# Gadersd/whisper-burn

Hardware: AMD Instinct MI355X
Metric: real-time factor (audio-sec/wall-sec) (higher is better)
Workload: dtype f32; 1 GPU; tiny.en, 30 s of 16 kHz audio per GPU per step, reference windowing (3 windows <= 14.9 s, 3 s overlap), HIP mel + encoder + KV-cached decode, greedy (beam_size 1), max_depth 100; windows=3, beam_size=1, max_depth=100, encoder_gemm_after_the_run=f16x3, parallelism=windows sharded over 1 GPU(s), 1 token all-gather

## Files before the change

### profiles/ps_timeline.py

```python
#!/usr/bin/env python3
import sys

import numpy as np

raw = np.fromfile(sys.argv[1], dtype=np.uint8)
n_steps, n_roles, grid, ns = [int(x) for x in raw[:16].view(np.int32)]
kinds = raw[16:16 + 4 * n_roles].view(np.int32)
n_st = 8 * n_steps * n_roles * ns
st = raw[16 + 4 * n_roles:16 + 4 * n_roles + n_st].view(np.uint64).reshape(n_steps, n_roles, ns).astype(np.float64)
tail = raw[16 + 4 * n_roles + n_st:]
block = None
if len(tail) >= 4 * (grid + 2) and int(tail[:4].view(np.int32)[0]) == 0x66664f52:
    role_off = tail[4:4 * (grid + 2)].view(np.int32)
    block = np.searchsorted(role_off, np.arange(n_roles), side="right") - 1
st[st == 0] = np.nan
names = {0: "attn", 1: "cross", 2: "mlp", 3: "logits", 4: "merge", 5: "finln"}
kind, layer, row = kinds & 0xff, (kinds >> 8) & 0xff, kinds >> 16
ran = ~np.isnan(st[:, :, 6])
last = int(np.nonzero(ran.any(1))[0].max()) + 1 if ran.any() else 0
lo = int(sys.argv[2]) if len(sys.argv) > 2 else min(8, max(last - 1, 0))
hi = int(sys.argv[3]) if len(sys.argv) > 3 else last
live_row = int(sys.argv[4]) if len(sys.argv) > 4 else 0
tick = 0.01
print(f"steps stamped {last} of {n_steps}, roles/step {n_roles}, grid {grid}; statistics over steps [{lo}, {hi}), attention roles of row {live_row}")
# ... 13 lines not shown
            continue
        s = sel[:, cols, :]
        def d(a, b):
            x = (s[:, :, b] - s[:, :, a]) * tick
            return np.nanmean(x) if np.isfinite(x).any() else float("nan")
        rel_done = np.nanmean((np.nanmax(s[:, :, 6], axis=1) - step_start) * tick)
        rel_arr = np.nanmean((np.nanmax(s[:, :, 7], axis=1) - step_start) * tick)
        nm = names[k] + (f" L{l}" if k < 3 else "")
        if k in (0, 1, 3, 4, 5):
            wp = np.nanmean((s[:, :, 1] - step_start[:, None]) * tick, axis=0)
            dn = np.nanmean((s[:, :, 6] - step_start[:, None]) * tick, axis=0)
            spread.append((nm, wp, dn, block[cols] if block is not None else None))
        print(f"{nm:<10}{int(cols.sum()):>4}{d(0,1):>8.2f}{d(1,2):>8.2f}{d(2,3):>8.2f}{d(3,4):>8.2f}{d(4,5):>8.2f}{d(5,6):>9.2f}{d(6,7):>8.2f}{d(1,6):>8.2f}{rel_done:>9.2f}{rel_arr:>9.2f}")
dd = np.diff(step_end) * tick
print(f"step time (merge arrived -> next merge arrived): mean {np.nanmean(dd):.2f} us, median {np.nanmedian(dd):.2f}, min {np.nanmin(dd):.2f}, max {np.nanmax(dd):.2f}")
print("over the roles of a kind (each role: mean over the steps), us after the step start (merge: of its own step's start):")
print(f"{'role':<10}{'n':>4}  {'wait passed @  min / median / max':<36}{'done @  min / median / max':<34}")
for nm, wp, dn, blk in spread:
    f3 = lambda v: f"{np.nanmin(v):8.2f} /{np.nanmedian(v):8.2f} /{np.nanmax(v):8.2f}"
    print(f"{nm:<10}{len(wp):>4}  {f3(wp):<36}{f3(dn):<34}")
    if nm == "logits" and blk is not None:
        late = np.argsort(-np.nan_to_num(dn))[:12]
        def held(b):
            o = [names[kind[i]] + f" L{layer[i]}" for i in np.nonzero(block == b)[0] if kind[i] < 3]
            return "+".join(o) if o else "-"
        print(f"{'':<10}last to finish (block [its layer roles]: wait passed @ / done @)  " +
              "  ".join(f"b{blk[i]}[{held(blk[i])}]:{wp[i]:.2f}/{dn[i]:.2f}" for i in late))
        behind = np.array([held(b) != "-" for b in blk])
        for lab, m in (("behind a layer role", behind), ("on blocks without one", ~behind)):
            if m.any():
# ... 5 lines not shown
```

### whisper-burn_amd/csrc/decode.h

```cpp
#pragma once
#include <hip/hip_runtime.h>
#include <hip/hip_ext.h>
#include <stdint.h>

#include <algorithm>
#include <vector>

#include "kernels.h"
#include "wb_internal.h"

namespace wb {

constexpr int MAX_BEAMS = 8;
constexpr int TOPK_MAX = 8;
constexpr int CA_STRIDE = 66;
constexpr int CA_NCH_MAX = 12;
constexpr int TS_STRIDE = 2 + 2 * TOPK_MAX;
constexpr int GV_CT = 128;
constexpr int GV_CT_LOGITS = 128;
constexpr int KS_MAX = 16;

enum { ST_N = 0, ST_STEP = 1, ST_HDR = 4 };
enum { GC_STEP = 0, GC_NDONE = 1, GC_ALLDONE = 2, GC_BAD = 3, GC_HDR = 4 };
struct StepLayout {
// ... 308 lines not shown
  const PsRole* roles = nullptr; int n_roles = 0;
  const int* role_off = nullptr;
  const int* res_role = nullptr;
  int n_logits_roles = 0;
  int n_layer = 0, n_rows = 0, S = 0, d = 0, n_head = 0, nb_mlp = 0;
  int n_pass = 1;
  int* ctl = nullptr;
  int step0 = 0, n_steps = 0;
  int n_forced = 0; int forced[PS_MAX_FORCED] = {0, 0, 0, 0, 0, 0, 0, 0};
  int mask_until_len = 0;
  const void* x_fin = nullptr; const void* P2 = nullptr; const float* b2_last = nullptr;
  void* g_xn = nullptr;
  unsigned tag_base = 0;
  const float* ln_g = nullptr; const float* ln_b = nullptr; float ln_eps = 0.f; int ln_inside = 0;
  const float* Et = nullptr; int vocab_ld = 0, V = 0; const float* mask = nullptr;
  float* tstats = nullptr; int n_tiles = 0;
  int* gctl = nullptr; int* gtok = nullptr; int Lmax = 0, eot = 0;
  const float* E = nullptr; const float* pos = nullptr; void* x0 = nullptr; int* tabs = nullptr;
  int* dead = nullptr;
  unsigned long long* stamps = nullptr;
};
enum { PS_DEAL_SLACK = 0, PS_DEAL_LEGACY = 1 };
struct PsDeal {
  std::vector<PsRole> roles;
  std::vector<int> role_off;
  std::vector<int> res_role;
  int n_lg = 0, n_res = 0;
};
PsDeal ps_deal_roles(int n_layer, int n_head, int n_rows, int nb_mlp, int n_tiles, int grid, int policy, bool res_on);
int ps_ctl_ints(int S, int n_layer);
bool dec_persist_supported(int d, int n_rows, int max_keys);
int dec_persist_resident_slots(int d, int n_rows, int max_keys);
bool dec_persist_resident_geometry(int d, int n_rows, int max_keys, int out[5]);
int dec_persist_max_grid(int device, int d, int n_rows, int max_keys);
int launch_dec_persist(hipStream_t st, const PersistArgs& a, int grid);
void launch_ps_seed(hipStream_t st, const float* x, int n, void* gx, unsigned tag, int* ctl);

#if defined(HIPEMU) && !defined(HIPEMU_PROD_GEOMETRY)
constexpr int CROSS_FUSED_MAX_C = 384;
#else
constexpr int CROSS_FUSED_MAX_C = 768;
#endif
constexpr int CROSS_FUSED_MAX_PASSES = 2;
void launch_dec_cross_fused(hipStream_t st, const CrossFusedArgs& a, int n_rows_hint);
bool dec_fused_supported(int d);
int dec_mlp_fused_planes(int d);
void launch_dec_mlp_fused(hipStream_t st, const MlpFusedArgs& a, int n_rows_hint);
void launch_dec_attn_fused(hipStream_t st, const AttnFusedArgs& a, int n_rows_hint);
int launch_dec_attn_fused_rounds(hipStream_t st, const AttnFusedArgs& a, int n_rows_hint, int n_reg);

}
// ... 1 lines not shown
```

### whisper-burn_amd/csrc/decode_chain.cpp

```cpp
#include <climits>
#include <cstring>
#include <string>

#include "decode_step.h"
#include "handoff.h"
#include "switches.h"

using namespace wb;

namespace wb {

struct PsPin { size_t seed, err, gctl, tok, total, ctl_ints; };
static PsPin ps_pin_layout(size_t ctl_ints, size_t tok_ints) {
  PsPin p;
  p.seed = 0; p.err = (ctl_ints + 3) & ~(size_t)3; p.gctl = p.err + 4; p.tok = p.gctl + ((ctl_ints + 3) & ~(size_t)3);
  p.total = p.tok + tok_ints; p.ctl_ints = ctl_ints;
  return p;
}
static int ps_pin_ensure(wb_session* s, size_t ints) {
  if (s->ps_pin_ints >= ints) return WB_OK;
  if (s->ps_pin_busy) { WB_HIP(hipStreamSynchronize(s->st)); s->ps_pin_busy = false; }
  if (s->ps_pin) { (void)hipHostFree(s->ps_pin); s->ps_pin = nullptr; s->ps_pin_ints = 0; }
  WB_HIP(hipHostMalloc((void**)&s->ps_pin, ints * 4, hipHostMallocDefault));
  s->ps_pin_ints = ints;
// ... 180 lines not shown
  WB_REQUIRE(n_forced >= 0 && n_forced <= PS_MAX_FORCED, WB_ERR_ARG, "persistent decode: %d prompt steps", n_forced);
  const char* inject = sw::persist_inject_fail();
  wb_model* m = s->m;
  const wb_dims& D = m->dims;
  const int d = D.n_text_state, H = D.n_text_head, NL = D.n_text_layer, V = D.n_vocab, S = s->S, W = s->W;
  const StepLayout& L = s->lay;
  hipStream_t st = s->st;
  const int NB = dec_mlp_fused_planes(d);
  const int n_tiles = (V + 127) / 128;
  WB_REQUIRE(NB <= 32 && H <= 8, WB_ERR_SHAPE, "persistent decode: more planes than its folds hold");
  WB_TRY(s->ps_gx.ensure_zeroed(((size_t)2 * S + 8) * d * 8, st));
  WB_TRY(s->ps_gpa.ensure_zeroed(((size_t)H * S + 8) * d * 8, st));
  WB_TRY(s->ps_gpc.ensure_zeroed(((size_t)H * S + 8) * d * 8, st));
  WB_TRY(s->ps_gp2.ensure_zeroed(((size_t)NB * S + 8) * d * 8, st));
  WB_TRY(s->ps_gxn.ensure_zeroed(((size_t)S + 8) * d * 8, st));
  if (((s->ps_launches + 1) & 0xffffu) == 0) {
    for (DevMem* b : {&s->ps_gx, &s->ps_gpa, &s->ps_gpc, &s->ps_gp2, &s->ps_gxn}) WB_HIP(hipMemsetAsync(b->p, 0, b->bytes, st));
    s->ps_launches++;
  }
  const unsigned tag_base = ((++s->ps_launches) & 0xffffu) << 16;
  char* gxb[2] = {static_cast<char*>(s->ps_gx.p), static_cast<char*>(s->ps_gx.p) + (size_t)S * d * 8};
  const char* res_sw = sw::persist_resident();
  const bool res_on = !(res_sw && res_sw[0] == '0') && dec_persist_resident_slots(d, W, s->maxC) > 0;
  bool built = false;
  WB_TRY(ps_setup_ensure(s, res_on, &built));
  const std::vector<PsRole>& roles = s->ps_roles_host;
  const int grid = s->ps_setup_grid, n_res = s->ps_setup_n_res;
  if (res_sw && !strcmp(res_sw, "log")) fprintf(stderr, "persist resident blocks: %d of %d\n", n_res, grid);
  const int n_ctl = ps_ctl_ints(S, NL);
  WB_TRY(s->ps_ctl.ensure((size_t)n_ctl * 4));
  WB_TRY(s->ps_dead.ensure((size_t)S * 4));
  WB_TRY(s->ps_tstats.ensure((size_t)S * n_tiles * 2 * 4));
  WB_HIP(hipMemsetAsync(s->ps_ctl.p, 0, (size_t)n_ctl * 4, st));
  WB_HIP(hipMemsetAsync(s->ps_dead.p, 0, (size_t)S * 4, st));
  PersistArgs a;
  a.layers = s->ps_layers.as<PsLayerArgs>(); a.roles = s->ps_roles.as<PsRole>(); a.n_roles = (int)roles.size();
  a.role_off = reinterpret_cast<const int*>(static_cast<char*>(s->ps_roles.p) + roles.size() * sizeof(PsRole));
  if (n_res > 0) a.res_role = a.role_off + (grid + 1);
  a.n_logits_roles = s->ps_setup_n_lg;
  a.n_layer = NL; a.n_rows = W; a.S = S; a.d = d; a.n_head = H; a.nb_mlp = NB;
  a.n_pass = s->maxC > CROSS_FUSED_MAX_C ? 2 : 1;
  a.ctl = s->ps_ctl.as<int>(); a.step0 = s->step; a.n_steps = n_forced + max_depth; a.mask_until_len = mask_until_len;
  a.n_forced = n_forced;
  for (int i = 0; i < n_forced; i++) a.forced[i] = forced[i];
  a.g_xn = s->ps_gxn.p;
  a.x_fin = gxb[(3 * NL) & 1]; a.P2 = s->ps_gp2.p; a.b2_last = m->dec[NL - 1].mlp2.b; a.tag_base = tag_base;
  a.ln_g = m->ln_dec.g; a.ln_b = m->ln_dec.b; a.ln_eps = m->ln_dec.eps; a.ln_inside = m->ln_eps_inside_sqrt;
  a.Et = m->tok_emb_t; a.vocab_ld = m->vocab_ld; a.V = V; a.mask = s->mask.as<float>();
  a.tstats = s->ps_tstats.as<float>(); a.n_tiles = n_tiles;
  a.gctl = s->gctl.as<int>(); a.gtok = s->gtok.as<int>(); a.Lmax = s->Lmax; a.eot = eot;
  a.E = m->tok_emb; a.pos = m->dec_pos; a.x0 = gxb[0]; a.tabs = s->tabs.as<int>(); a.dead = s->ps_dead.as<int>();
  const char* stamps_path = sw::ps_stamps();
  const size_t n_stamps = stamps_path ? (size_t)(n_forced + max_depth) * roles.size() * 8 : 0;
  if (n_stamps) {
    WB_TRY(s->ps_stamps.ensure(n_stamps * 8));
    WB_HIP(hipMemsetAsync(s->ps_stamps.p, 0, n_stamps * 8, st));
    a.stamps = s->ps_stamps.as<unsigned long long>();
  }
  WB_REQUIRE(3 * NL * (n_forced + max_depth + 1) + 4 < 0x10000, WB_ERR_SHAPE,
             "persistent decode: %d layers x %d steps do not fit the 16-bit granule tags", NL, max_depth);
  launch_dec_prepare(st, reinterpret_cast<const int*>(s->host_block_dev), s->state.as<int>(), L, W, s->tabs.as<int>(),
                     s->Lmax, m->tok_emb, m->dec_pos, d, s->x.as<float>(), s->gctl.as<int>());
  launch_ps_seed(st, s->x.as<float>(), W * d, gxb[0], tag_base + 1u, s->ps_ctl.as<int>());
  hipEvent_t e0 = nullptr, e1 = nullptr;
// ... 286 lines not shown
```

### whisper-burn_amd/csrc/decode_fused_bodies.h

```cpp
#pragma once
#include <hip/hip_runtime.h>

#include "decode.h"
#include "handoff.h"
#include "wave_ops.h"

namespace wb {
namespace fused {

struct PsStep {
  const unsigned* ctr = nullptr; unsigned target = 0; int ctr_index = 0;
  const int* ctl = nullptr;
  int step = 0;
  int n_rows = 0;
  const int* dead = nullptr;
  int* lds_flag = nullptr;
  unsigned long long* stamp = nullptr;
  int n_ctr = 1;
  unsigned tag_in = 0, tag_out = 0;
  bool known_dead = false;
  mutable bool saw_dead = false;
};
constexpr int PS_STAMPS = 8;
__device__ __forceinline__ void ps_stamp(const PsStep& ps, int k) {
#ifdef WB_EXP_FINE
  if (k == 4 || k == 5) return;
#endif
  if (ps.stamp && threadIdx.x == 0) ps.stamp[k] = wall_clock64();
}
__device__ __forceinline__ void ps_stamp_fine(const PsStep& ps, int k) {
#ifdef WB_EXP_FINE
  if (ps.stamp && threadIdx.x == 0) ps.stamp[k] = wall_clock64();
#endif
}
__device__ __forceinline__ bool ps_wait(const PsStep& ps) {
  const bool ok = ps.n_ctr > 1 ? hx_wait_same(ps.ctr, ps.target, ps.n_ctr, ps.ctl, ps.step, ps.ctr_index, ps.lds_flag)
// ... 11 lines not shown
  }
  __builtin_amdgcn_s_sleep(1);
  return false;
}
__device__ __forceinline__ bool ps_sweeps_ok(const PsStep& ps) { return *ps.lds_flag != 0; }
template <int UNITS>
__device__ __forceinline__ void ps_nap() {
#if !defined(WB_PS_DRY) || defined(WB_PS_DRY_NAPS)
#ifndef WB_PS_NAP_ADJ
#define WB_PS_NAP_ADJ 0
#endif
#pragma unroll
  for (int i = 0; i < UNITS + (WB_PS_NAP_ADJ); i++) __builtin_amdgcn_s_sleep(64);
#endif
}

#ifdef WB_STAMPS
#define WB_STAMP_DECL unsigned long long stamp_buf[16];
#define WB_STAMP(i) do { if (threadIdx.x == 0 && blockIdx.x == 0 && blockIdx.y == 0) sm.stamp_buf[i] = wall_clock64(); } while (0)
#define WB_STAMP_FLUSH(a, n) do { if (threadIdx.x == 0 && blockIdx.x == 0 && blockIdx.y == 0 && (a).stamps) for (int _i = 0; _i < (n); _i++) (a).stamps[_i] = sm.stamp_buf[_i]; } while (0)
#else
#define WB_STAMP_DECL
#define WB_STAMP(i) do {} while (0)
#define WB_STAMP_FLUSH(a, n) do {} while (0)
#endif

constexpr int FD_MAX = 512;
constexpr int FA_MAXPOS = 448;


// ... 595 lines not shown
      if (NIT > 1) load_round(wr[1], 1);
      if constexpr (NREG == 4) {
        const int it2 = (RG::NRND > 0 && res != nullptr) ? 2 + RG::NRND : 2;
        load_round(wr[2], it2);
        load_round(wr[3], it2 + 1);
      }
      if constexpr (PS && NREG == 2) { if (tid < 192) qbias = gld(a.bqkv + (tid >> 6) * d + h * 64 + (tid & 63)); }
    };
    if constexpr (PS) {
#if !defined(WB_PS_DRY)
      if (!ps.known_dead) {
        load_weights();
        if constexpr (NREG == 2) load_cache_tile();
      }
#endif
      if (!ps_wait(ps)) return false;
      dead = ps.known_dead ? 1 : ld_i<true>(ps.dead + r);
      if (r >= n_rows || dead) { ps.saw_dead = true; return true; }
      const Buf16 xgb(a.g_x_in), pgb(a.g_pend);
      const uint32_t pvo = (uint32_t)(r * d + c);
      const int iplane = a.S * d;
      if (a.KSp > 0) ps_nap<2>();
      constexpr int FP = 4 * DPL;
      float v = 0.f, accp = a.KSp > 0 ? gld(a.pbias + c) : 0.f;
      unsigned sweeps = 0;
      Gran gx{0u, 0.f}, g[FP];
#pragma unroll
      for (int j = 0; j < FP; j++) g[j] = Gran{0u, 0.f};
      for (;;) {
        if (gx.tag != ps.tag_in) gx = ld_gran(xgb, pvo, 0u);
        if (a.KSp > 0) {
#pragma unroll
          for (int j = 0; j < FP; j++)
            if (j < a.KSp && g[j].tag != ps.tag_in) g[j] = ld_gran(pgb, pvo, (uint32_t)(j * iplane));
        }
        bool ok = gx.tag == ps.tag_in;
        if (a.KSp > 0) {
#pragma unroll
          for (int j = 0; j < FP; j++) ok &= (j >= a.KSp) || g[j].tag == ps.tag_in;
        }
        if (ok) {
          v = gx.v;
          if (a.KSp > 0) {
#pragma unroll
            for (int j = 0; j < FP; j++) accp += (j < a.KSp) ? g[j].v : 0.f;
            v += accp;
          }
          break;
        }
        if (ps_sweep_retry(sweeps, ps)) { *ps.lds_flag = 0; break; }
      }
      xfold = v;
      if (tid < d) hs[tid] = v;
#if !defined(WB_PS_DRY)
      if constexpr (NREG == 4) {
        load_cache_tile();
        if (tid < 192) qbias = gld(a.bqkv + (tid >> 6) * d + h * 64 + (tid & 63));
      }
#endif
    } else {
    float v = a.x_in[(int64_t)r * d + c];
    constexpr int FP = 32;
    float t[FP];
    float accp = 0.f;
    if (a.KSp > 0) {
// ... 356 lines not shown
    const float* pp = a.pend + (int64_t)r * d + c;
    const int64_t plane = (int64_t)a.S * d;
    if constexpr (PS) {
#if !defined(WB_PS_DRY)
      if (!ps.known_dead) {
        load_weights();
        load_keys();
      }
#endif
      if (!ps_wait(ps)) return false;
      dead = ps.known_dead ? 1 : ld_i<true>(ps.dead + r);
      if (r >= n_live || dead) { ps.saw_dead = true; return true; }
      const Buf16 xgb(a.g_x_in), pgb(a.g_pend);
      const uint32_t pvo = (uint32_t)(r * d + c);
      const int iplane = a.S * d;
      ps_nap<4>();
      constexpr int FP = 8;
      float v = 0.f, accp = gld(a.pbias + c);
      unsigned sweeps = 0;
      Gran gx{0u, 0.f}, g[FP];
#pragma unroll
      for (int j = 0; j < FP; j++) g[j] = Gran{0u, 0.f};
      for (;;) {
        if (gx.tag != ps.tag_in) gx = ld_gran(xgb, pvo, 0u);
#pragma unroll
        for (int j = 0; j < FP; j++)
          if (j < a.KSp && g[j].tag != ps.tag_in) g[j] = ld_gran(pgb, pvo, (uint32_t)(j * iplane));
        bool ok = gx.tag == ps.tag_in;
#pragma unroll
        for (int j = 0; j < FP; j++) ok &= (j >= a.KSp) || g[j].tag == ps.tag_in;
        if (ok) {
// ... 246 lines not shown
```

### whisper-burn_amd/csrc/decode_persist.hip

```cpp
#include <hip/hip_runtime.h>

#include <climits>
#include <vector>

#include "decode.h"
#include "decode_fused_bodies.h"
#include "handoff.h"
#include "wave_ops.h"

namespace wb {
namespace {

using namespace fused;

constexpr int PS_NT = 512;
constexpr int PS_CT = 128;
constexpr int PS_NGO = 16;

template <int DPL>
struct FinLnLds { alignas(16) float hs[64 * DPL]; };
template <int DPL>
__device__ __forceinline__ bool ps_finln_role(const PersistArgs& a, const int r, const PsStep& ps, FinLnLds<DPL>& sm) {
  constexpr int d = 64 * DPL, FP = 4 * DPL;
  auto& hs = sm.hs;
// ... 37 lines not shown
    ln_stats_lds<DPL>(hs, d, lane, a.ln_eps, a.ln_inside, mean, denom);
    const Buf16 xo(a.g_xn);
    st_gran(xo, (uint32_t)(r * d + tid), ps.tag_out, (v - mean) / denom * g_own + b_own);
  }
  return true;
}

template <int MR, int DPL>
struct LogitsLds {
  alignas(16) float xs[MR][64 * DPL];
  alignas(16) float red[8][MR][PS_CT];
  float tilev[MR][PS_CT];
};
template <int MR, int DPL>
__device__ __forceinline__ bool ps_logits_role(const PersistArgs& a, const int tile0, const int n_t, const PsStep& ps,
                                               const bool forced, LogitsLds<MR, DPL>& sm) {
  constexpr int d = 64 * DPL, NT = PS_NT, CT = PS_CT;
  constexpr int NR = d / 16;
  constexpr int EPT = (MR * d + NT - 1) / NT;
  constexpr int PCH = EPT <= 3 ? 8 : EPT <= 6 ? 4 : 2;
  constexpr int NQ = MR * CT / NT;
  constexpr bool TWO = DPL <= 6;
  auto& xs = sm.xs; auto& red = sm.red; auto& tilev = sm.tilev;
  const int tid = role_tid<true>(), lane = tid & 63, wave = tid >> 6;
  const int hh = lane >> 5, c4 = (lane & 31) * 4;
  const Buf16 etb(a.Et);
  auto load_tile = [&](float4 (&w)[NR], int tile) {
    const int n0 = tile * CT;
    const bool col_ok = n0 + c4 < a.vocab_ld;
    const uint32_t vo = (uint32_t)((2 * wave + hh) * NR * a.vocab_ld + n0 + (col_ok ? c4 : 0));
#pragma unroll
// ... 38 lines not shown
      if (ps_sweep_retry(sweeps, ps)) { *ps.lds_flag = 0; break; }
    }
#pragma unroll
    for (int i = 0; i < EPT; i++) {
      const int e = tid + NT * i;
      if (e < MR * d) (&xs[0][0])[e] = v[i];
    }
  }
  ps_stamp(ps, 2);
  __syncthreads();
  if (!ps_sweeps_ok(ps)) return false;
  ps_stamp(ps, 3);
  if (forced) return true;
#if defined(WB_PS_DRY)
  for (int t = 0; t < n_t; t++)
    if (wave < MR && !((deadm >> wave) & 1) && lane == 0) {
      float* ts = a.tstats + ((int64_t)wave * a.n_tiles + tile0 + t) * 2;
      st_f<true>(ts, 0.f);
      st_f<true>(ts + 1, __int_as_float((tile0 + t) * CT));
    }
  return true;
#endif
  auto run_tile = [&](const float4 (&w)[NR], int tile) {
    const int n0 = tile * CT;
    float mk[NQ];
#pragma unroll
    for (int q = 0; q < NQ; q++) {
      const int col = n0 + ((tid + NT * q) & (CT - 1));
      mk[q] = (use_mask && col < a.V) ? a.mask[col] : 0.f;
    }
    float acc[MR][4];
#pragma unroll
    for (int r = 0; r < MR; r++) { acc[r][0] = acc[r][1] = acc[r][2] = acc[r][3] = 0.f; }
#pragma unroll
// ... 24 lines not shown
      const int e = tid + NT * q, r = e / CT, c = e & (CT - 1);
      float v = 0.f;
#pragma unroll
      for (int w8 = 0; w8 < 8; w8++) v += red[w8][r][c];
      v += mk[q];
      if (n0 + c >= a.V) v = -INFINITY;
      tilev[r][c] = v;
    }
    __syncthreads();
    if (wave < MR && !((deadm >> wave) & 1)) {
      const int r = wave;
      const float v0 = tilev[r][lane], v1 = tilev[r][lane + 64];
      float bvv; int bi;
      if (better(v0, lane, v1, lane + 64)) { bvv = v0; bi = lane; } else { bvv = v1; bi = lane + 64; }
      wave_argmax(bvv, bi);
      if (lane == 0) {
        float* ts = a.tstats + ((int64_t)r * a.n_tiles + tile) * 2;
        st_f<true>(ts, bvv);
        st_f<true>(ts + 1, __int_as_float(n0 + bi));
      }
    }
  };
  run_tile(w0, tile0);
  ps_stamp(ps, 4);
  if constexpr (TWO) {
    if (n_t > 1) run_tile(w1, tile0 + 1);
    ps_stamp(ps, 5);
    for (int t = 2; t < n_t; t++) { load_tile(w0, tile0 + t); run_tile(w0, tile0 + t); }
  } else {
    for (int t = 1; t < n_t; t++) { load_tile(w0, tile0 + t); run_tile(w0, tile0 + t); }
  }
  return true;
}

struct MergeLds { float redv[8]; int redi[8]; unsigned tgt[8]; };
// ... 5 lines not shown
  {
    auto& tgt = sm.tgt;
    if (tid < 8) tgt[tid] = (unsigned)(e + 1) * (unsigned)n_per_ctr[tid];
    __syncthreads();
    if (!hx_wait_many(clog, tgt, 8, ps.ctl, ps.step, 1000, ps.lds_flag)) return false;
  }
  ps_stamp(ps, 1);
  const int len = ps.step + 1;
  const int fin_now = ld_i<true>(a.dead + r);
  const int tok_prev = ld_i<true>(a.gctl + GC_HDR + r);
  int gi;
  if (e < a.n_forced) {
    gi = a.forced[e];
  } else {
    float bv = -INFINITY; int bi = 0x7fffffff;
    for (int t = tid; t < a.n_tiles; t += PS_NT) {
      const float* ts = a.tstats + ((int64_t)r * a.n_tiles + t) * 2;
      const float v = ld_f<true>(ts);
      const int id = __float_as_int(ld_f<true>(ts + 1));
      if (better(v, id, bv, bi)) { bv = v; bi = id; }
    }
    wave_argmax(bv, bi);
    if (lane == 0) { redv[wave] = bv; redi[wave] = bi; }
    __syncthreads();
    float gv = redv[0]; gi = redi[0];
#pragma unroll
    for (int j = 1; j < 8; j++)
      if (better(redv[j], redi[j], gv, gi)) { gv = redv[j]; gi = redi[j]; }
    if ((unsigned)gi >= 0x7fffffffu) { gi = a.eot; if (tid == 0) a.gctl[GC_BAD] = 1; }
  }
  const int finished = fin_now || (gi == a.eot && e >= a.n_forced);
  const int tok_next = fin_now ? tok_prev : gi;
  if (tid == 0 && !fin_now) {
    st_i_sc1(a.gctl + GC_HDR + r, gi);
    a.gtok[r * a.Lmax + len] = gi;
// ... 76 lines not shown
    else if (role.kind == PSR_CROSS) dec_cross_res_fill<DPL, NP, RS>(a.layers[role.layer].cross, role.a, role.b, res_buf);
  }
  unsigned long long dead_seen = 0;
  for (int e = 0; e < a.n_steps; e++) {
    for (int i = i_lo; i < i_hi; i++) {
      const PsRole role = a.roles[i];
      PsStep ps;
      ps.known_dead = i - i_lo < 64 && ((dead_seen >> (i - i_lo)) & 1ull) != 0;
      ps.ctl = a.ctl; ps.step = a.step0 + e; ps.n_rows = R; ps.dead = a.dead; ps.lds_flag = &wait_flag[0];
      unsigned long long* stp = a.stamps ? a.stamps + ((size_t)e * a.n_roles + i) * PS_STAMPS : nullptr;
      if (stp && threadIdx.x == 0) stp[0] = wall_clock64();
      ps.stamp = stp;
      int out;
      bool ok;
      const unsigned tag_l = a.tag_base + 2u + 3u * (unsigned)(e * NL + (role.kind <= PSR_MLP ? role.layer : NL - 1));
      if (role.kind == PSR_ATTN) {
        const AttnFusedArgs la = a.layers[role.layer].attn;
        if (role.layer == 0) { ps.ctr_index = C_X + role.b; ps.target = (unsigned)e; }
        else { ps.ctr_index = C_CROSS + role.layer - 1; ps.target = (unsigned)(e + 1) * H * R; }
        ps.ctr = cptr(ps.ctr_index);
        ps.tag_out = tag_l; ps.tag_in = tag_l - 1u;
        ok = dec_attn_body<DPL, true, RS>(la, role.a, role.b, ps, lds.attn, i == res_i ? res_buf : nullptr);
        out = C_ATTN + role.layer * S + role.b;
      } else if (role.kind == PSR_CROSS) {
        const CrossFusedArgs la = a.layers[role.layer].cross;
        if (role.layer == 0) { ps.ctr_index = C_X + role.b; ps.target = (unsigned)e; }
        else { ps.ctr_index = C_MLP + role.layer - 1; ps.target = (unsigned)(e + 1) * NB; }
        ps.ctr = cptr(ps.ctr_index);
        ps.tag_out = tag_l + 1u; ps.tag_in = tag_l;
        ok = dec_cross_body<DPL, true, NP, RS>(la, role.a, role.b, ps, lds.cross, i == res_i ? res_buf : nullptr);
        out = C_CROSS + role.layer;
      } else if (role.kind == PSR_MLP) {
        const MlpFusedArgs la = a.layers[role.layer].mlp;
        ps.ctr_index = C_ATTN + role.layer * S; ps.target = (unsigned)(e + 1) * H; ps.n_ctr = R;
        ps.ctr = cptr(ps.ctr_index);
        ps.tag_out = tag_l + 2u; ps.tag_in = tag_l + 1u;
        ok = dec_mlp_body<MR, DPL, false, true>(la, role.a, ps, lds.mlp);
        out = C_MLP + role.layer;
      } else if (role.kind == PSR_FINLN) {
        ps.ctr_index = C_CROSS + NL - 1; ps.target = (unsigned)(e + 1) * H * R;
        ps.ctr = cptr(ps.ctr_index);
        ps.tag_in = tag_l + 2u; ps.tag_out = tag_l + 2u;
        ok = ps_finln_role<DPL>(a, role.b, ps, lds.finln);
        out = C_GO + PS_NGO;
      } else if (role.kind == PSR_LOGITS) {
        ps.ctr_index = C_GO + (role.layer % PS_NGO); ps.target = (unsigned)(e + 1);
        ps.ctr = cptr(ps.ctr_index);
        ps.tag_in = tag_l + 2u;
        ok = ps_logits_role<MR, DPL>(a, role.a, role.b, ps, e < a.n_forced, lds.logits);
        out = C_LOG + (role.layer & 7);
      } else {
        ok = ps_merge_role(a, role.b, e, ps, cptr(C_LOG), n_per_ctr, lds.merge);
        out = C_X + role.b;
      }
      if (!ok) return;
      if (ps.saw_dead && i - i_lo < 64) dead_seen |= 1ull << (i - i_lo);
      if (stp && threadIdx.x == 0) stp[6] = wall_clock64();
      if (role.kind == PSR_CROSS && role.layer == NL - 1)
        hx_arrive_broadcast(cptr(out), (unsigned)(e + 1) * H * R, cptr(C_GO), PS_NGO, (unsigned)(e + 1));
      else
        hx_arrive(cptr(out));
      if (stp && threadIdx.x == 0) stp[7] = wall_clock64();
    }
  }
}

__global__ void ps_seed_kernel(const float* __restrict__ x, int n, void* gx, unsigned tag, int* ctl) {
  if (blockIdx.x == 0 && threadIdx.x == 0) ctl[HX_STOP] = INT_MAX;
  const Buf16 b(gx);
  for (int i = blockIdx.x * blockDim.x + threadIdx.x; i < n; i += gridDim.x * blockDim.x) st_gran(b, (uint32_t)i, tag, x[i]);
}

template <int DPL, int MR, int NP>
int max_blocks_per_cu() {
  int nb = 0;
  if (hipOccupancyMaxActiveBlocksPerMultiprocessor(&nb, (dec_persist_kernel<DPL, MR, NP>), PS_NT, 0) != hipSuccess) return 0;
  return nb;
}

}

int dec_persist_resident_slots(int d, int n_rows, int max_keys) {
  if (!dec_persist_supported(d, n_rows, max_keys)) return 0;
  const int dpl = d / 64, mr = n_rows > 4 ? 8 : 4, np = max_keys > CROSS_FUSED_MAX_C ? 2 : 1;
#define WB_PS_SLOTS(DPL_, MR_, NP_) \
// ... 36 lines not shown
  int per = 0;
  const bool big = n_rows > 4;
  if (max_keys > CROSS_FUSED_MAX_C)
    per = d == 128 ? max_blocks_per_cu<2, 4, 2>() : d == 384 ? max_blocks_per_cu<6, 4, 2>() : max_blocks_per_cu<8, 4, 2>();
  else if (d == 128) per = big ? max_blocks_per_cu<2, 8, 1>() : max_blocks_per_cu<2, 4, 1>();
  else if (d == 384) per = big ? max_blocks_per_cu<6, 8, 1>() : max_blocks_per_cu<6, 4, 1>();
  else per = max_blocks_per_cu<8, 4, 1>();
  if (per <= 0) return 0;
  return cus * 1;
}

void launch_ps_seed(hipStream_t st, const float* x, int n, void* gx, unsigned tag, int* ctl) {
  hipLaunchKernelGGL(ps_seed_kernel, dim3((n + 255) / 256), dim3(256), 0, st, x, n, gx, tag, ctl);
}

int launch_dec_persist(hipStream_t st, const PersistArgs& a, int grid) {
  const dim3 g(grid), b(PS_NT);
  const bool big = a.n_rows > 4;
  hipError_t e = hipErrorInvalidValue;
#define WB_PS(DPL_, MR_, NP_) e = WB_LAUNCH_COOP((dec_persist_kernel<DPL_, MR_, NP_>), g, b, 0, st, a)
  if (a.n_pass > 1) {
    if (big) return -1;
    if (a.d == 128) WB_PS(2, 4, 2); else if (a.d == 384) WB_PS(6, 4, 2); else if (a.d == 512) WB_PS(8, 4, 2);
  }
  else if (a.d == 128) { if (big) WB_PS(2, 8, 1); else WB_PS(2, 4, 1); }
  else if (a.d == 384) { if (big) WB_PS(6, 8, 1); else WB_PS(6, 4, 1); }
  else if (a.d == 512 && !big) WB_PS(8, 4, 1);
#undef WB_PS
  return e == hipSuccess ? 0 : -1;
}
// ... 3 lines not shown
```

### whisper-burn_amd/csrc/handoff.h

```cpp
#pragma once
#include <hip/hip_runtime.h>
#include <stdint.h>

namespace wb {

#ifndef WB_DRAIN_VMEM
#define WB_DRAIN_VMEM() asm volatile("s_waitcnt vmcnt(0)" ::: "memory")
#endif
#ifndef WB_LAUNCH_COOP
#define WB_LAUNCH_COOP(kernel, grid, block, shmem, stream, arg) \
  [&]() { void* _args[] = {(void*)&(arg)}; return hipLaunchCooperativeKernel((const void*)(kernel), grid, block, _args, shmem, stream); }()
#endif

#ifndef WB_PIN_F4
#define WB_PIN_F4(v) asm volatile("" : "+v"((v).x), "+v"((v).y), "+v"((v).z), "+v"((v).w) : : "memory")
#endif
#ifndef WB_LAUNDER_V
#define WB_LAUNDER_V(x) asm volatile("" : "+v"(x))
#endif
template <bool PS>
__device__ __forceinline__ int role_tid() {
  int t = threadIdx.x;
  if constexpr (PS) WB_LAUNDER_V(t);
  return t;
// ... 71 lines not shown
__device__ __forceinline__ Gran ld_gran(const Buf16& b, uint32_t gran_voff, uint32_t gran_soff) {
  const hx_u32x2 u = __builtin_amdgcn_raw_buffer_load_b64(b.r, gran_voff * 8u, gran_soff * 8u, 16);
  return Gran{u[0], __uint_as_float(u[1])};
}
__device__ __forceinline__ void st_gran(const Buf16& b, uint32_t gran_off, unsigned tag, float v) {
  hx_u32x2 u; u[0] = tag; u[1] = __float_as_uint(v);
  __builtin_amdgcn_raw_buffer_store_b64(u, b.r, gran_off * 8u, 0, 16);
}
__device__ __forceinline__ void st_gran4(const Buf16& b, uint32_t gran_off, unsigned tag, float4 v) {
  hx_u32x4 u;
  u[0] = tag; u[1] = __float_as_uint(v.x); u[2] = tag; u[3] = __float_as_uint(v.y);
  __builtin_amdgcn_raw_buffer_store_b128(u, b.r, gran_off * 8u, 0, 16);
  u[1] = __float_as_uint(v.z); u[3] = __float_as_uint(v.w);
  __builtin_amdgcn_raw_buffer_store_b128(u, b.r, gran_off * 8u + 16u, 0, 16);
}
constexpr unsigned HX_SWEEP_LIMIT = 1u << 20;

constexpr unsigned HX_SPIN_LIMIT = 4u * 1000u * 1000u;

constexpr int HX_LINE = 32;
enum { HX_STOP = 0,
       HX_ERR = HX_LINE,
       HX_NDONE = 2 * HX_LINE,
       HX_HDR = 3 * HX_LINE };

__device__ __forceinline__ void hx_arrive(unsigned* ctr) {
  WB_DRAIN_VMEM();
  __syncthreads();
  if (threadIdx.x == 0) __hip_atomic_fetch_add(ctr, 1u, __ATOMIC_RELAXED, __HIP_MEMORY_SCOPE_AGENT);
}
// ... 9 lines not shown
           __hip_atomic_load(ctl + HX_ERR, __ATOMIC_RELAXED, __HIP_MEMORY_SCOPE_AGENT) != 0)) { ok = 0; break; }
      if (++spins > HX_SPIN_LIMIT) {
        __hip_atomic_store(const_cast<int*>(ctl) + HX_ERR, 1 + ctr_index, __ATOMIC_RELAXED, __HIP_MEMORY_SCOPE_AGENT);
        ok = 0;
        break;
      }
      __builtin_amdgcn_s_sleep(2);
    }
    if (ok && __hip_atomic_load(ctl + HX_STOP, __ATOMIC_RELAXED, __HIP_MEMORY_SCOPE_AGENT) <= step) ok = 0;
    *lds_flag = ok;
  }
  __syncthreads();
  const int ok = *lds_flag;
  __syncthreads();
  return ok != 0;
}

__device__ __forceinline__ bool hx_wait_many(const unsigned* ctr, const unsigned* target, int n, const int* ctl, int step,
                                             int ctr_index, int* lds_flag) {
  if (threadIdx.x < 64) {
    const int lane = threadIdx.x;
    const bool mine = lane < n;
    const unsigned tgt = mine ? target[lane] : 0u;
    int ok = 1;
    unsigned spins = 0;
    for (;;) {
      const bool have = !mine || __hip_atomic_load(ctr + lane * HX_LINE, __ATOMIC_RELAXED, __HIP_MEMORY_SCOPE_AGENT) >= tgt;
      if (__ballot(!have) == 0ull) break;
      if ((spins & 15u) == 15u &&
          (__hip_atomic_load(ctl + HX_STOP, __ATOMIC_RELAXED, __HIP_MEMORY_SCOPE_AGENT) <= step ||
// ... 58 lines not shown
```

### whisper-burn_amd/csrc/switches.h

```cpp
#pragma once

namespace wb {
namespace sw {

enum Kind { DEFAULT_ON, OPT_IN, UNSET_OR_1, TRI, INT, STR };

#define WB_BOOL_SWITCHES(X)                                                                                                          \
  X(graph, "WHISPER_HIP_GRAPH", DEFAULT_ON, "on", "replay captured hipGraphs of the decode steps; 0: enqueue every step eagerly")    \
  X(chain, "WHISPER_HIP_CHAIN", DEFAULT_ON, "on", "device-chained greedy decode; 0: one host round trip per step")                   \
  X(beam_chain, "WHISPER_HIP_BEAM_CHAIN", DEFAULT_ON, "on", "beam bookkeeping on the device; 0: host-driven beam search")            \
  X(persist, "WHISPER_HIP_PERSIST", DEFAULT_ON, "on", "persistent flag-chained greedy kernel; 0: one launch per sublayer")           \
  X(persist_prefill, "WHISPER_HIP_PERSIST_PREFILL", DEFAULT_ON, "on", "the persistent launch runs the prompt itself; 0: host prefill") \
  X(prefill_pass, "WHISPER_HIP_PREFILL_PASS", DEFAULT_ON, "on", "a session's prefill mode 1 is honoured (one-pass prompt prefill); 0: steps everywhere") \
  X(poll, "WHISPER_HIP_POLL", DEFAULT_ON, "on", "chained greedy: spin on mapped progress flags; 0: copy + synchronise per chunk")    \
  X(speculate, "WHISPER_HIP_SPECULATE", OPT_IN, "off", "chained greedy: enqueue one segment ahead of the finished flags")            \
  X(fuse_sub, "WHISPER_HIP_FUSE_SUB", DEFAULT_ON, "on", "fused self-attention and MLP sublayer kernels; 0: per-matrix GEMVs")        \
  X(fuse_x, "WHISPER_HIP_FUSE_X", DEFAULT_ON, "on", "fused cross-attention sublayer kernel; 0: chunked cross-attention + GEMV")      \
  X(fuse_q, "WHISPER_HIP_FUSE_Q", DEFAULT_ON, "on", "chunked cross-attention blocks project their own queries")                      \
  X(fuse_co, "WHISPER_HIP_FUSE_CO", OPT_IN, "off", "chunked cross-attention blocks apply the out-projection too")                    \
  X(fuse16, "WHISPER_HIP_FUSE16", DEFAULT_ON, "on", "9 - 16 live rows stay on the fused sublayer kernels; 0: batch mode")            \
  X(batch_skinny, "WHISPER_HIP_BATCH_SKINNY", DEFAULT_ON, "on", "batch mode: skinny weight-stream GEMM up to 64 rows; 0: tiled GEMM") \
  X(cross_stream, "WHISPER_HIP_CROSS_STREAM", DEFAULT_ON, "on", "batch mode, one beam per window: streaming cross-attention")        \
  X(sk_pair, "WHISPER_HIP_SK_PAIR", OPT_IN, "off", "skinny GEMM: the waves' partial tiles meet pairwise")                            \
  X(mlp16_mfma, "WHISPER_HIP_MLP16_MFMA", DEFAULT_ON, "on", "9 - 16-row fused MLP on the matrix cores; 0: two row groups of 8")      \
// ... 7 lines not shown
  X(attn_kvsplit, "WHISPER_HIP_ATTN_KVSPLIT", DEFAULT_ON, "on", "encoder attention splits long key ranges across blocks")            \
  X(gpu_turn, "WHISPER_HIP_GPU_TURN", DEFAULT_ON, "on", "one entry point at a time per device and process (developer: 0 drops it)")  \
  X(session_pool, "WHISPER_HIP_SESSION_POOL", DEFAULT_ON, "on", "released sessions are parked for reuse; 0: freed (developer A/B)")  \
  X(pcm_stage, "WHISPER_HIP_PCM_STAGE", OPT_IN, "off", "host PCM is uploaded through a pinned per-session buffer")
#define WB_INT_SWITCHES(X)                                                                                                           \
  X(cross_stream_fuse, "WHISPER_HIP_CROSS_STREAM_FUSE", TRI, -1, "streaming cross-attention folds / projects its query; unset: d <= 768") \
  X(sk_max_blocks, "WHISPER_HIP_SK_MAX_BLOCKS", INT, 256, "skinny GEMM: most blocks a K-split may launch")                           \
  X(split_tile, "WHISPER_HIP_SPLIT_TILE", INT, 0, "split-precision GEMM: force a tile shape (developer A/B; 0: choose)")             \
  X(enc_trace_extra, "WHISPER_HIP_ENC_TRACE_EXTRA", INT, 0, "bit mask of extra stages in the encoder trace (1 pcm, 2 mel, 4 maxima)")
#define WB_STR_SWITCHES(X)                                                                                                           \
  X(enc_trace, "WHISPER_HIP_ENC_TRACE", STR, nullptr, "directory for per-thread dumps of the encoder stages (developer)")            \
  X(ps_stamps, "WHISPER_HIP_PS_STAMPS", STR, nullptr, "file for the persistent kernel's role timeline (developer)")                  \
  X(persist_resident, "WHISPER_HIP_PERSIST_RESIDENT", STR, nullptr, "persistent kernel: step-invariant operands stay in LDS (on); 0: off; log: on + report") \
  X(persist_setup, "WHISPER_HIP_PERSIST_SETUP", STR, nullptr, "persistent kernel: launch setup cached on the session (on); 0: built per call; log: on + report; 0log: both") \
  X(persist_deal, "WHISPER_HIP_PERSIST_DEAL", STR, nullptr, "persistent kernel: merge / final-LN roles kept off the first-layer attention blocks (on); legacy: the least loaded blocks; log: on + report") \
  X(persist_inject_fail, "WHISPER_HIP_PERSIST_INJECT_FAIL", STR, nullptr, "test hook: \"launch\" = the cooperative launch is refused")

#define WB_SW_DECL(fn, name, kind, dflt, what) bool fn();
WB_BOOL_SWITCHES(WB_SW_DECL)
#undef WB_SW_DECL
#define WB_SW_DECL(fn, name, kind, dflt, what) int fn();
WB_INT_SWITCHES(WB_SW_DECL)
#undef WB_SW_DECL
#define WB_SW_DECL(fn, name, kind, dflt, what) const char* fn();
WB_STR_SWITCHES(WB_SW_DECL)
#undef WB_SW_DECL

}
}
```

Before: 2534 x real-time.

## Let first-layer attention pick the next token from tagged tile records

Logits tiles now write tagged 16-byte records into a double-buffered array. Each first-layer self-attention block scans these records and takes the argmax itself, then builds the next embedding directly. This removes the wait for the merge role's row on the step-to-step critical path. The cross-attention nap is also shortened on that path. The cost is that every first-layer attention block redundantly reads all tile records, and a new two-counter wait adds a fallback path, so correctness relies on the tag protocol.

```diff
diff --git a/profiles/ps_timeline.py b/profiles/ps_timeline.py
--- a/profiles/ps_timeline.py
+++ b/profiles/ps_timeline.py
@@ -51,6 +51,12 @@
         print(f"{nm:<10}{int(cols.sum()):>4}{d(0,1):>8.2f}{d(1,2):>8.2f}{d(2,3):>8.2f}{d(3,4):>8.2f}{d(4,5):>8.2f}{d(5,6):>9.2f}{d(6,7):>8.2f}{d(1,6):>8.2f}{rel_done:>9.2f}{rel_arr:>9.2f}")
 dd = np.diff(step_end) * tick
 print(f"step time (merge arrived -> next merge arrived): mean {np.nanmean(dd):.2f} us, median {np.nanmedian(dd):.2f}, min {np.nanmin(dd):.2f}, max {np.nanmax(dd):.2f}")
+a0 = (kind == 0) & (layer == 0) & (row == live_row)
+if a0.any() and (kind == 3).any() and hi - lo > 1:
+    lg_done = np.nanmax(st[lo:hi - 1][:, kind == 3, 6], axis=1)
+    for nm, red in (("first", np.nanmin), ("last", np.nanmax)):
+        edge = (red(st[lo + 1:hi][:, a0, 2], axis=1) - lg_done) * tick
+        print(f"last logits done -> attn L0 p2 ({nm} block of row {live_row}): mean {np.nanmean(edge):.2f} us, median {np.nanmedian(edge):.2f}, min {np.nanmin(edge):.2f}, max {np.nanmax(edge):.2f}")
 print("over the roles of a kind (each role: mean over the steps), us after the step start (merge: of its own step's start):")
 print(f"{'role':<10}{'n':>4}  {'wait passed @  min / median / max':<36}{'done @  min / median / max':<34}")
 for nm, wp, dn, blk in spread:
diff --git a/whisper-burn_amd/csrc/decode.h b/whisper-burn_amd/csrc/decode.h
--- a/whisper-burn_amd/csrc/decode.h
+++ b/whisper-burn_amd/csrc/decode.h
@@ -346,7 +346,8 @@
   unsigned tag_base = 0;
   const float* ln_g = nullptr; const float* ln_b = nullptr; float ln_eps = 0.f; int ln_inside = 0;
   const float* Et = nullptr; int vocab_ld = 0, V = 0; const float* mask = nullptr;
-  float* tstats = nullptr; int n_tiles = 0;
+  void* tstats = nullptr; int n_tiles = 0;
+  int pick = 1;
   int* gctl = nullptr; int* gtok = nullptr; int Lmax = 0, eot = 0;
   const float* E = nullptr; const float* pos = nullptr; void* x0 = nullptr; int* tabs = nullptr;
   int* dead = nullptr;
@@ -367,6 +368,7 @@
 int dec_persist_max_grid(int device, int d, int n_rows, int max_keys);
 int launch_dec_persist(hipStream_t st, const PersistArgs& a, int grid);
 void launch_ps_seed(hipStream_t st, const float* x, int n, void* gx, unsigned tag, int* ctl);
+void launch_ps_pick_test(hipStream_t st, const void* rec, int n_tiles, unsigned tag, int* ctl, int* out_id);
 
 #if defined(HIPEMU) && !defined(HIPEMU_PROD_GEOMETRY)
 constexpr int CROSS_FUSED_MAX_C = 384;
diff --git a/whisper-burn_amd/csrc/decode_chain.cpp b/whisper-burn_amd/csrc/decode_chain.cpp
--- a/whisper-burn_amd/csrc/decode_chain.cpp
+++ b/whisper-burn_amd/csrc/decode_chain.cpp
@@ -218,8 +218,9 @@
   WB_TRY(s->ps_gpc.ensure_zeroed(((size_t)H * S + 8) * d * 8, st));
   WB_TRY(s->ps_gp2.ensure_zeroed(((size_t)NB * S + 8) * d * 8, st));
   WB_TRY(s->ps_gxn.ensure_zeroed(((size_t)S + 8) * d * 8, st));
+  WB_TRY(s->ps_tstats.ensure_zeroed((size_t)2 * S * n_tiles * 16, st));
   if (((s->ps_launches + 1) & 0xffffu) == 0) {
-    for (DevMem* b : {&s->ps_gx, &s->ps_gpa, &s->ps_gpc, &s->ps_gp2, &s->ps_gxn}) WB_HIP(hipMemsetAsync(b->p, 0, b->bytes, st));
+    for (DevMem* b : {&s->ps_gx, &s->ps_gpa, &s->ps_gpc, &s->ps_gp2, &s->ps_gxn, &s->ps_tstats}) WB_HIP(hipMemsetAsync(b->p, 0, b->bytes, st));
     s->ps_launches++;
   }
   const unsigned tag_base = ((++s->ps_launches) & 0xffffu) << 16;
@@ -234,7 +235,6 @@
   const int n_ctl = ps_ctl_ints(S, NL);
   WB_TRY(s->ps_ctl.ensure((size_t)n_ctl * 4));
   WB_TRY(s->ps_dead.ensure((size_t)S * 4));
-  WB_TRY(s->ps_tstats.ensure((size_t)S * n_tiles * 2 * 4));
   WB_HIP(hipMemsetAsync(s->ps_ctl.p, 0, (size_t)n_ctl * 4, st));
   WB_HIP(hipMemsetAsync(s->ps_dead.p, 0, (size_t)S * 4, st));
   PersistArgs a;
@@ -251,7 +251,9 @@
   a.x_fin = gxb[(3 * NL) & 1]; a.P2 = s->ps_gp2.p; a.b2_last = m->dec[NL - 1].mlp2.b; a.tag_base = tag_base;
   a.ln_g = m->ln_dec.g; a.ln_b = m->ln_dec.b; a.ln_eps = m->ln_dec.eps; a.ln_inside = m->ln_eps_inside_sqrt;
   a.Et = m->tok_emb_t; a.vocab_ld = m->vocab_ld; a.V = V; a.mask = s->mask.as<float>();
-  a.tstats = s->ps_tstats.as<float>(); a.n_tiles = n_tiles;
+  a.tstats = s->ps_tstats.p; a.n_tiles = n_tiles;
+  const char* pick_sw = sw::persist_pick();
+  a.pick = pick_sw && !strcmp(pick_sw, "merge") ? 0 : 1;
   a.gctl = s->gctl.as<int>(); a.gtok = s->gtok.as<int>(); a.Lmax = s->Lmax; a.eot = eot;
   a.E = m->tok_emb; a.pos = m->dec_pos; a.x0 = gxb[0]; a.tabs = s->tabs.as<int>(); a.dead = s->ps_dead.as<int>();
   const char* stamps_path = sw::ps_stamps();
diff --git a/whisper-burn_amd/csrc/decode_fused_bodies.h b/whisper-burn_amd/csrc/decode_fused_bodies.h
--- a/whisper-burn_amd/csrc/decode_fused_bodies.h
+++ b/whisper-burn_amd/csrc/decode_fused_bodies.h
@@ -20,6 +20,10 @@
   unsigned tag_in = 0, tag_out = 0;
   bool known_dead = false;
   mutable bool saw_dead = false;
+  const void* pk_rec = nullptr; int pk_n_tiles = 0; unsigned pk_tag = 0;
+  const unsigned* pk_go = nullptr; unsigned pk_go_target = 0;
+  const float* pk_E = nullptr; const float* pk_pos = nullptr; int pk_eot = 0;
+  bool cross_early = false;
 };
 constexpr int PS_STAMPS = 8;
 __device__ __forceinline__ void ps_stamp(const PsStep& ps, int k) {
@@ -61,6 +65,44 @@
   for (int i = 0; i < UNITS + (WB_PS_NAP_ADJ); i++) __builtin_amdgcn_s_sleep(64);
 #endif
 }
+
+constexpr int PS_PICK_NONE = 0x7fffffff;
+#ifdef WB_PS_PICK_NOINLINE
+__device__ __attribute__((noinline)) int ps_pick_token(
+#else
+__device__ __forceinline__ int ps_pick_token(
+#endif
+const void* rec, const int n_tiles, const unsigned tag, const PsStep& ps,
+                                             float* xch, const int tid) {
+  const Buf16 rb(rec);
+  float bv = -INFINITY; int bi = PS_PICK_NONE;
+  unsigned sweeps = 0;
+  for (int t = tid; t < n_tiles;) {
+    const Rec q = ld_rec(rb, (uint32_t)t);
+    if (q.t0 == tag && q.t1 == tag) {
+      if (better(q.v, q.id, bv, bi)) { bv = q.v; bi = q.id; }
+      t += 512;
+    } else if (ps_sweep_retry(sweeps, ps)) {
+      *ps.lds_flag = 0;
+      break;
+    }
+  }
+  wave_argmax(bv, bi);
+  int* xid = reinterpret_cast<int*>(xch) + 8;
+  if ((tid & 63) == 0) { xch[tid >> 6] = bv; xid[tid >> 6] = bi; }
+  __syncthreads();
+  float gv = xch[0]; int gi = xid[0];
+#pragma unroll
+  for (int j = 1; j < 8; j++)
+    if (better(xch[j], xid[j], gv, gi)) { gv = xch[j]; gi = xid[j]; }
+  return gi;
+}
+#ifndef WB_PS_PICK_NAP
+#define WB_PS_PICK_NAP 6
+#endif
+#ifndef WB_PS_CROSS0_NAP
+#define WB_PS_CROSS0_NAP 1
+#endif
 
 #ifdef WB_STAMPS
 #define WB_STAMP_DECL unsigned long long stamp_buf[16];
@@ -686,6 +728,24 @@
         if constexpr (NREG == 2) load_cache_tile();
       }
 #endif
+      float v = 0.f;
+      bool picked = false;
+      if (ps.pk_rec != nullptr && !ps.known_dead) {
+        const int go = hx_wait_two(ps.pk_go, ps.pk_go_target, ps.ctr, ps.target - 1u, ps.ctl, ps.step, ps.ctr_index, ps.lds_flag,
+                                   ps.dead + (r < n_rows ? r : 0));
+        if (go == 0) return false;
+        ps_stamp(ps, 1);
+        if (r < n_rows && go == 1) {
+          ps_nap<WB_PS_PICK_NAP>();
+          const int tok = ps_pick_token(ps.pk_rec, ps.pk_n_tiles, ps.pk_tag, ps, red, tid);
+          if (!ps_sweeps_ok(ps)) return false;
+          if (tok != PS_PICK_NONE && tok != ps.pk_eot) {
+            v = gld(ps.pk_E + (int64_t)tok * d + c) + gld(ps.pk_pos + c);
+            picked = true;
+          }
+        }
+      }
+      if (!picked) {
       if (!ps_wait(ps)) return false;
       dead = ps.known_dead ? 1 : ld_i<true>(ps.dead + r);
       if (r >= n_rows || dead) { ps.saw_dead = true; return true; }
@@ -694,7 +754,7 @@
       const int iplane = a.S * d;
       if (a.KSp > 0) ps_nap<2>();
       constexpr int FP = 4 * DPL;
-      float v = 0.f, accp = a.KSp > 0 ? gld(a.pbias + c) : 0.f;
+      float accp = a.KSp > 0 ? gld(a.pbias + c) : 0.f;
       unsigned sweeps = 0;
       Gran gx{0u, 0.f}, g[FP];
 #pragma unroll
@@ -721,6 +781,7 @@
           break;
         }
         if (ps_sweep_retry(sweeps, ps)) { *ps.lds_flag = 0; break; }
+      }
       }
       xfold = v;
       if (tid < d) hs[tid] = v;
@@ -1107,7 +1168,7 @@
       const Buf16 xgb(a.g_x_in), pgb(a.g_pend);
       const uint32_t pvo = (uint32_t)(r * d + c);
       const int iplane = a.S * d;
-      ps_nap<4>();
+      if (ps.cross_early) ps_nap<WB_PS_CROSS0_NAP>(); else ps_nap<4>();
       constexpr int FP = 8;
       float v = 0.f, accp = gld(a.pbias + c);
       unsigned sweeps = 0;
diff --git a/whisper-burn_amd/csrc/decode_persist.hip b/whisper-burn_amd/csrc/decode_persist.hip
--- a/whisper-burn_amd/csrc/decode_persist.hip
+++ b/whisper-burn_amd/csrc/decode_persist.hip
@@ -75,7 +75,7 @@
 };
 template <int MR, int DPL>
 __device__ __forceinline__ bool ps_logits_role(const PersistArgs& a, const int tile0, const int n_t, const PsStep& ps,
-                                               const bool forced, LogitsLds<MR, DPL>& sm) {
+                                               const bool forced, const int par, LogitsLds<MR, DPL>& sm) {
   constexpr int d = 64 * DPL, NT = PS_NT, CT = PS_CT;
   constexpr int NR = d / 16;
   constexpr int EPT = (MR * d + NT - 1) / NT;
@@ -144,10 +144,9 @@
   if (forced) return true;
 #if defined(WB_PS_DRY)
   for (int t = 0; t < n_t; t++)
-    if (wave < MR && !((deadm >> wave) & 1) && lane == 0) {
-      float* ts = a.tstats + ((int64_t)wave * a.n_tiles + tile0 + t) * 2;
-      st_f<true>(ts, 0.f);
-      st_f<true>(ts + 1, __int_as_float((tile0 + t) * CT));
+    if (wave < MR && !((deadm >> wave) & 1)) {
+      const int r_u = __builtin_amdgcn_readfirstlane(wave);
+      if (lane == 0) st_rec(Buf16(a.tstats), (uint32_t)((par * a.S + r_u) * a.n_tiles + tile0 + t), ps.tag_in, 0.f, (tile0 + t) * CT);
     }
   return true;
 #endif
@@ -202,11 +201,8 @@
       float bvv; int bi;
       if (better(v0, lane, v1, lane + 64)) { bvv = v0; bi = lane; } else { bvv = v1; bi = lane + 64; }
       wave_argmax(bvv, bi);
-      if (lane == 0) {
-        float* ts = a.tstats + ((int64_t)r * a.n_tiles + tile) * 2;
-        st_f<true>(ts, bvv);
-        st_f<true>(ts + 1, __int_as_float(n0 + bi));
-      }
+      const int r_u = __builtin_amdgcn_readfirstlane(r);
+      if (lane == 0) st_rec(Buf16(a.tstats), (uint32_t)((par * a.S + r_u) * a.n_tiles + tile), ps.tag_in, bvv, n0 + bi);
     }
   };
   run_tile(w0, tile0);
@@ -242,11 +238,10 @@
     gi = a.forced[e];
   } else {
     float bv = -INFINITY; int bi = 0x7fffffff;
+    const Buf16 recb(a.tstats);
     for (int t = tid; t < a.n_tiles; t += PS_NT) {
-      const float* ts = a.tstats + ((int64_t)r * a.n_tiles + t) * 2;
-      const float v = ld_f<true>(ts);
-      const int id = __float_as_int(ld_f<true>(ts + 1));
-      if (better(v, id, bv, bi)) { bv = v; bi = id; }
+      const Rec q = ld_rec(recb, (uint32_t)(((e & 1) * a.S + r) * a.n_tiles + t));
+      if (better(q.v, q.id, bv, bi)) { bv = q.v; bi = q.id; }
     }
     wave_argmax(bv, bi);
     if (lane == 0) { redv[wave] = bv; redi[wave] = bi; }
@@ -353,12 +348,20 @@
       int out;
       bool ok;
       const unsigned tag_l = a.tag_base + 2u + 3u * (unsigned)(e * NL + (role.kind <= PSR_MLP ? role.layer : NL - 1));
+      const bool pick_e = a.pick != 0 && e >= 1 && e - 1 >= a.n_forced && ps.step < a.Lmax;
       if (role.kind == PSR_ATTN) {
         const AttnFusedArgs la = a.layers[role.layer].attn;
         if (role.layer == 0) { ps.ctr_index = C_X + role.b; ps.target = (unsigned)e; }
         else { ps.ctr_index = C_CROSS + role.layer - 1; ps.target = (unsigned)(e + 1) * H * R; }
         ps.ctr = cptr(ps.ctr_index);
         ps.tag_out = tag_l; ps.tag_in = tag_l - 1u;
+        if (role.layer == 0 && pick_e) {
+          ps.pk_rec = static_cast<const char*>(a.tstats) + ((size_t)((e - 1) & 1) * S + role.b) * a.n_tiles * sizeof(Rec);
+          ps.pk_n_tiles = a.n_tiles;
+          ps.pk_tag = a.tag_base + 4u + 3u * (unsigned)((e - 1) * NL + NL - 1);
+          ps.pk_go = cptr(C_GO + (role.b * H + role.a) % PS_NGO); ps.pk_go_target = (unsigned)e;
+          ps.pk_E = a.E; ps.pk_pos = a.pos + (int64_t)ps.step * a.d; ps.pk_eot = a.eot;
+        }
         ok = dec_attn_body<DPL, true, RS>(la, role.a, role.b, ps, lds.attn, i == res_i ? res_buf : nullptr);
         out = C_ATTN + role.layer * S + role.b;
       } else if (role.kind == PSR_CROSS) {
@@ -367,6 +370,7 @@
         else { ps.ctr_index = C_MLP + role.layer - 1; ps.target = (unsigned)(e + 1) * NB; }
         ps.ctr = cptr(ps.ctr_index);
         ps.tag_out = tag_l + 1u; ps.tag_in = tag_l;
+        ps.cross_early = role.layer == 0 && pick_e;
         ok = dec_cross_body<DPL, true, NP, RS>(la, role.a, role.b, ps, lds.cross, i == res_i ? res_buf : nullptr);
         out = C_CROSS + role.layer;
       } else if (role.kind == PSR_MLP) {
@@ -386,7 +390,7 @@
         ps.ctr_index = C_GO + (role.layer % PS_NGO); ps.target = (unsigned)(e + 1);
         ps.ctr = cptr(ps.ctr_index);
         ps.tag_in = tag_l + 2u;
-        ok = ps_logits_role<MR, DPL>(a, role.a, role.b, ps, e < a.n_forced, lds.logits);
+        ok = ps_logits_role<MR, DPL>(a, role.a, role.b, ps, e < a.n_forced, e & 1, lds.logits);
         out = C_LOG + (role.layer & 7);
       } else {
         ok = ps_merge_role(a, role.b, e, ps, cptr(C_LOG), n_per_ctr, lds.merge);
@@ -408,6 +412,17 @@
   if (blockIdx.x == 0 && threadIdx.x == 0) ctl[HX_STOP] = INT_MAX;
   const Buf16 b(gx);
   for (int i = blockIdx.x * blockDim.x + threadIdx.x; i < n; i += gridDim.x * blockDim.x) st_gran(b, (uint32_t)i, tag, x[i]);
+}
+
+__global__ __launch_bounds__(PS_NT) void ps_pick_test_kernel(const void* rec, int n_tiles, unsigned tag, int* ctl, int* out_id) {
+  __shared__ float xch[16];
+  __shared__ int flag;
+  PsStep ps;
+  ps.ctl = ctl; ps.step = -1; ps.lds_flag = &flag;
+  if (threadIdx.x == 0) flag = 1;
+  __syncthreads();
+  const int tok = ps_pick_token(rec, n_tiles, tag, ps, xch, role_tid<true>());
+  if (threadIdx.x == 0) *out_id = ps_sweeps_ok(ps) ? tok : -1;
 }
 
 template <int DPL, int MR, int NP>
@@ -474,6 +489,10 @@
   hipLaunchKernelGGL(ps_seed_kernel, dim3((n + 255) / 256), dim3(256), 0, st, x, n, gx, tag, ctl);
 }
 
+void launch_ps_pick_test(hipStream_t st, const void* rec, int n_tiles, unsigned tag, int* ctl, int* out_id) {
+  hipLaunchKernelGGL(ps_pick_test_kernel, dim3(1), dim3(PS_NT), 0, st, rec, n_tiles, tag, ctl, out_id);
+}
+
 int launch_dec_persist(hipStream_t st, const PersistArgs& a, int grid) {
   const dim3 g(grid), b(PS_NT);
   const bool big = a.n_rows > 4;
diff --git a/whisper-burn_amd/csrc/handoff.h b/whisper-burn_amd/csrc/handoff.h
--- a/whisper-burn_amd/csrc/handoff.h
+++ b/whisper-burn_amd/csrc/handoff.h
@@ -109,6 +109,16 @@
   u[1] = __float_as_uint(v.z); u[3] = __float_as_uint(v.w);
   __builtin_amdgcn_raw_buffer_store_b128(u, b.r, gran_off * 8u + 16u, 0, 16);
 }
+struct Rec { unsigned t0; float v; unsigned t1; int id; };
+__device__ __forceinline__ Rec ld_rec(const Buf16& b, uint32_t rec_off) {
+  const hx_u32x4 u = __builtin_amdgcn_raw_buffer_load_b128(b.r, rec_off * 16u, 0, 16);
+  return Rec{u[0], __uint_as_float(u[1]), u[2], (int)u[3]};
+}
+__device__ __forceinline__ void st_rec(const Buf16& b, uint32_t rec_off, unsigned tag, float v, int id) {
+  hx_u32x4 u;
+  u[0] = tag; u[1] = __float_as_uint(v); u[2] = tag; u[3] = (unsigned)id;
+  __builtin_amdgcn_raw_buffer_store_b128(u, b.r, 0, rec_off * 16u, 16);
+}
 constexpr unsigned HX_SWEEP_LIMIT = 1u << 20;
 
 constexpr unsigned HX_SPIN_LIMIT = 4u * 1000u * 1000u;
@@ -148,6 +158,35 @@
   const int ok = *lds_flag;
   __syncthreads();
   return ok != 0;
+}
+
+__device__ __forceinline__ int hx_wait_two(const unsigned* c0, unsigned t0, const unsigned* c1, unsigned t1, const int* ctl,
+                                           int step, int ctr_index, int* lds_flag, const int* word) {
+  if (threadIdx.x == 0) {
+    int ok = 1;
+    unsigned spins = 0;
+    bool have0 = false;
+    for (;;) {
+      if (!have0) have0 = __hip_atomic_load(c0, __ATOMIC_RELAXED, __HIP_MEMORY_SCOPE_AGENT) >= t0;
+      if (have0 && __hip_atomic_load(c1, __ATOMIC_RELAXED, __HIP_MEMORY_SCOPE_AGENT) >= t1) break;
+      if ((spins & 15u) == 15u &&
+          (__hip_atomic_load(ctl + HX_STOP, __ATOMIC_RELAXED, __HIP_MEMORY_SCOPE_AGENT) <= step ||
+           __hip_atomic_load(ctl + HX_ERR, __ATOMIC_RELAXED, __HIP_MEMORY_SCOPE_AGENT) != 0)) { ok = 0; break; }
+      if (++spins > HX_SPIN_LIMIT) {
+        __hip_atomic_store(const_cast<int*>(ctl) + HX_ERR, 1 + ctr_index, __ATOMIC_RELAXED, __HIP_MEMORY_SCOPE_AGENT);
+        ok = 0;
+        break;
+      }
+      __builtin_amdgcn_s_sleep(2);
+    }
+    if (ok && __hip_atomic_load(ctl + HX_STOP, __ATOMIC_RELAXED, __HIP_MEMORY_SCOPE_AGENT) <= step) ok = 0;
+    if (ok && __hip_atomic_load(word, __ATOMIC_RELAXED, __HIP_MEMORY_SCOPE_AGENT) != 0) ok = 2;
+    *lds_flag = ok;
+  }
+  __syncthreads();
+  const int ok = *lds_flag;
+  __syncthreads();
+  return ok;
 }
 
 __device__ __forceinline__ bool hx_wait_many(const unsigned* ctr, const unsigned* target, int n, const int* ctl, int step,
diff --git a/whisper-burn_amd/csrc/switches.h b/whisper-burn_amd/csrc/switches.h
--- a/whisper-burn_amd/csrc/switches.h
+++ b/whisper-burn_amd/csrc/switches.h
@@ -45,6 +45,7 @@
   X(persist_resident, "WHISPER_HIP_PERSIST_RESIDENT", STR, nullptr, "persistent kernel: step-invariant operands stay in LDS (on); 0: off; log: on + report") \
   X(persist_setup, "WHISPER_HIP_PERSIST_SETUP", STR, nullptr, "persistent kernel: launch setup cached on the session (on); 0: built per call; log: on + report; 0log: both") \
   X(persist_deal, "WHISPER_HIP_PERSIST_DEAL", STR, nullptr, "persistent kernel: merge / final-LN roles kept off the first-layer attention blocks (on); legacy: the least loaded blocks; log: on + report") \
+  X(persist_pick, "WHISPER_HIP_PERSIST_PICK", STR, nullptr, "persistent kernel: first-layer self-attention picks the next token from the tile records itself (on); merge: it waits for the merge role's row") \
   X(persist_inject_fail, "WHISPER_HIP_PERSIST_INJECT_FAIL", STR, nullptr, "test hook: \"launch\" = the cooperative launch is refused")
 
 #define WB_SW_DECL(fn, name, kind, dflt, what) bool fn();
```

After: 2598 x real-time (median of 6 runs). +2.6%, better.
